# DigITs-AIML/MMNN_STS

Hardware: AMD Instinct MI355X
Metric: training volumes/sec/GPU (128^3 T1+T2+preop, batch 2) at 1/2/4/8 MI355X (higher is better)
Workload: dtype f32; 1 GPU; configs[2] --images --preop --survival --blend: MultiModalModel(DenseNet121-3D(in=2), MLP(32), blend) fwd + GradientBlender Cox loss + bwd + grad all-reduce + SGD-Nesterov/OneCycle step, dropout 0.2; micro_batch=2, global_batch=2, tabular=32, parallelism=dp1, allreduce=none

## Files before the change

### mmnn_sts_amd/csrc/densenet.hip

```cpp
#include "densenet.hpp"

#include <string.h>

#include <algorithm>

#include "fprop.hpp"
#include "stem.hpp"
#include "wgrad.hpp"

namespace mmnn {

constexpr size_t KZ_PART_BYTES = (size_t)512 * 4 * 1024 * sizeof(float);
constexpr unsigned KZ_CNT_ENTRIES = 4096;

namespace {
struct Panel { const float* p; unsigned bytes; };
struct LayerBind {
  BnFwd bn1, bn2;
  BnBwd gr_new, gr_t1;
  StatPtr dg1, dg2, s_x;
  View x, g;
  View x_new, g_new;
  View t1, dz2;
};
}

static long conv1_elems(const Plan& p, int cin) { return (long)p.mid * cin; }
static long conv2_elems(const Plan& p) { return (long)p.cfg.growth * p.mid * 27; }
static long trans_elems(const TransOff& t) { return (long)t.cout * t.cin; }
static size_t conv2_split_bytes(const Plan& p) { return (size_t)3 * conv2_elems(p) * sizeof(uint16_t); }

int plan_build(Plan& p, const NetCfg& cfg, int N, int D, int H, int W) {
  MMNN_REQUIRE(cfg.nblocks >= 1 && cfg.nblocks <= MAX_BLOCKS, "plan: 1..%d dense blocks supported, got %d", MAX_BLOCKS, cfg.nblocks);
  MMNN_REQUIRE(cfg.in_channels >= 1 && cfg.in_channels <= 4, "plan: in_channels must be 1..4, got %d", cfg.in_channels);
  MMNN_REQUIRE(cfg.init_features >= 1 && cfg.init_features <= 64, "plan: init_features must be <= 64, got %d", cfg.init_features);
  MMNN_REQUIRE(cfg.growth >= 1 && cfg.growth <= 32, "plan: growth_rate must be <= 32, got %d", cfg.growth);
  MMNN_REQUIRE(cfg.bn_size >= 1 && cfg.dropout_p >= 0.f && cfg.dropout_p < 1.f, "plan: bad bn_size / dropout");
  MMNN_REQUIRE(N >= 1 && D >= 1 && H >= 1 && W >= 1, "plan: bad input extent");
  p.cfg = cfg; p.N = N; p.D = D; p.H = H; p.W = W;
  p.mid = cfg.bn_size * cfg.growth;
  p.D0 = (D - 1) / 2 + 1; p.H0 = (H - 1) / 2 + 1; p.W0 = (W - 1) / 2 + 1;
  int d = (p.D0 - 1) / 2 + 1, h = (p.H0 - 1) / 2 + 1, w = (p.W0 - 1) / 2 + 1;
  int c = cfg.init_features;
  for (int b = 0; b < cfg.nblocks; ++b) {
    MMNN_REQUIRE(cfg.block_layers[b] >= 1, "plan: empty dense block %d", b);
    MMNN_REQUIRE(d >= 1 && h >= 1 && w >= 1, "plan: input too small, block %d has no voxels", b + 1);
    p.Db[b] = d; p.Hb[b] = h; p.Wb[b] = w; p.Vb[b] = d * h * w;
    p.cin_b[b] = c;
    p.nrep_b[b] = (b == 0 || (long)N * d * h * w >= 32768) ? NREP : ((long)N * d * h * w >= 4096 ? 2 : 1);
    p.ctot_b[b] = c + cfg.block_layers[b] * cfg.growth;
    c = p.ctot_b[b];
    if (b != cfg.nblocks - 1) {
      MMNN_REQUIRE(c % 2 == 0, "plan: transition halves an odd channel count");
      c /= 2; d /= 2; h /= 2; w /= 2;
    }
  }
  long po = 0, ro = 0;
  int nbn = 0;
  auto bn = [&](int ch, long& w_, long& b_, long& m_, long& v_) { w_ = po; po += ch; b_ = po; po += ch; m_ = ro; ro += ch; v_ = ro; ro += ch; ++nbn; };
  p.p_conv0 = po; po += (long)cfg.init_features * cfg.in_channels * 343;
  bn(cfg.init_features, p.p_n0w, p.p_n0b, p.r_n0m, p.r_n0v);
  p.layers.assign(cfg.nblocks, {});
  p.trans.clear();
  for (int b = 0; b < cfg.nblocks; ++b) {
    int ci = p.cin_b[b];
    for (int l = 0; l < cfg.block_layers[b]; ++l) {
      LayerOff lo;
      lo.cin = ci;
      bn(ci, lo.n1w, lo.n1b, lo.r1m, lo.r1v);
      lo.c1 = po; po += conv1_elems(p, ci);
      bn(p.mid, lo.n2w, lo.n2b, lo.r2m, lo.r2v);
      lo.c2 = po; po += conv2_elems(p);
      p.layers[b].push_back(lo);
      ci += cfg.growth;
    }
    if (b != cfg.nblocks - 1) {
      TransOff t;
      t.cin = ci; t.cout = ci / 2;
      bn(ci, t.nw, t.nb, t.rm, t.rv);
      t.cw = po; po += trans_elems(t);
      p.trans.push_back(t);
    } else {
      bn(ci, p.p_n5w, p.p_n5b, p.r_n5m, p.r_n5v);
    }
  }
  p.n_params = po; p.n_runstats = ro; p.n_bn = nbn;

  Carver cv;
  const int nb = cfg.nblocks;
  const size_t F = sizeof(float);
  const long V0 = (long)p.D0 * p.H0 * p.W0;
  p.o_conv0 = cv.take((size_t)N * cfg.init_features * V0 * F);
  p.o_idx = cv.take((size_t)N * cfg.init_features * p.Vb[0]);
  p.o_t1.assign(nb, {});
  size_t dap = 0;
  for (int b = 0; b < nb; ++b) {
    p.o_x[b] = cv.take((size_t)N * p.ctot_b[b] * p.Vb[b] * F);
    p.o_g[b] = cv.take((size_t)N * p.ctot_b[b] * p.Vb[b] * F);
    for (int l = 0; l < cfg.block_layers[b]; ++l) p.o_t1[b].push_back(cv.take((size_t)N * p.mid * p.Vb[b] * F));
    if (b != nb - 1) {
      p.o_ap[b] = cv.take((size_t)N * p.ctot_b[b] * p.Vb[b + 1] * F);
      dap = std::max(dap, (size_t)N * p.ctot_b[b] * p.Vb[b + 1] * F);
    } else {
      p.o_ap[b] = 0;
    }
  }
  p.o_dap = cv.take(dap ? dap : 256);
  p.o_dz0 = cv.take((size_t)N * cfg.init_features * V0 * F);
  const size_t PAIR = 2 * NREP * sizeof(double);
  p.o_fstat = cv.cur;
  p.o_st_conv0 = cv.take(PAIR * cfg.init_features);
  p.o_st_t1.assign(nb, {});
  for (int b = 0; b < nb; ++b) {
    p.o_st_x[b] = cv.take(PAIR * p.ctot_b[b]);
    for (int l = 0; l < cfg.block_layers[b]; ++l) p.o_st_t1[b].push_back(cv.take(PAIR * p.mid));
  }
  p.fstat_bytes = cv.cur - p.o_fstat;
  p.o_bstat = cv.cur;
  p.o_dg_n0 = cv.take(PAIR * cfg.init_features);
  p.o_dg_n1.assign(nb, {}); p.o_dg_n2.assign(nb, {}); p.o_dg_tr.clear();
  for (int b = 0; b < nb; ++b) {
    p.o_s_x[b] = cv.take(PAIR * p.ctot_b[b]);
    for (int l = 0; l < cfg.block_layers[b]; ++l) {
      p.o_dg_n1[b].push_back(cv.take(PAIR * p.layers[b][l].cin));
      p.o_dg_n2[b].push_back(cv.take(PAIR * p.mid));
    }
    if (b != nb - 1) p.o_dg_tr.push_back(cv.take(PAIR * p.ctot_b[b]));
  }
  p.o_dg_n5 = cv.take(PAIR * p.ctot_b[nb - 1]);
  p.bstat_bytes = cv.cur - p.o_bstat;
  p.o_pk_conv0 = cv.take((size_t)7 * stem_krows(cfg.in_channels) * 64 * F);
  p.o_pk_c1.assign(nb, {}); p.o_pk_c2f.assign(nb, {}); p.o_pk_c2b.assign(nb, {}); p.o_pk_tr.clear();
  p.o_pk_c2f3.assign(nb, {}); p.o_pk_c2b3.assign(nb, {});
  p.x3_bytes = 0;
  for (int b = 0; b < nb; ++b) {
    FpropArgs f, g;
    memset(&f, 0, sizeof(f));
    f.N = N; f.D = p.Db[b]; f.H = p.Hb[b]; f.W = p.Wb[b];
    g = f;
    f.Cin = p.mid; f.M = cfg.growth;
    g.Cin = cfg.growth; g.M = p.mid;
    const bool f3 = conv3_fwd_bf16x3_eligible(f), b3 = conv3_dgrad_bf16x3_eligible(g);
    if (f3) p.x3_bytes = std::max(p.x3_bytes, conv3_bf16x3_plane_bytes(f));
    if (b3) p.x3_bytes = std::max(p.x3_bytes, conv3_bf16x3_plane_bytes(g));
    for (int l = 0; l < cfg.block_layers[b]; ++l) {
      p.o_pk_c1[b].push_back(cv.take(conv1_elems(p, p.layers[b][l].cin) * F));
      p.o_pk_c2f[b].push_back(cv.take(conv2_elems(p) * F));
      p.o_pk_c2b[b].push_back(cv.take(conv2_elems(p) * F));
      p.o_pk_c2f3[b].push_back(f3 ? cv.take(conv2_split_bytes(p)) : 0);
      p.o_pk_c2b3[b].push_back(b3 ? cv.take(conv2_split_bytes(p)) : 0);
    }
    if (b != nb - 1) p.o_pk_tr.push_back(cv.take(trans_elems(p.trans[b]) * F));
  }
  p.o_x3 = p.x3_bytes ? cv.take(p.x3_bytes) : 0;
  p.ns_conv0 = stem_wgrad_pick_splits(N, p.D0, p.H0, p.W0, cfg.in_channels);
  p.o_sl_conv0 = cv.take((size_t)p.ns_conv0 * cfg.in_channels * cfg.init_features * 352 * F);
  p.o_sl_c1.assign(nb, {}); p.o_sl_c2.assign(nb, {}); p.ns_c1.assign(nb, {}); p.ns_c2.assign(nb, {});
  p.o_sl_tr.clear(); p.ns_tr.clear();
  for (int b = 0; b < nb; ++b) {
    for (int l = 0; l < cfg.block_layers[b]; ++l) {
      const int ci = p.layers[b][l].cin;
      int pairs = 0;
      {
        const int cw = wgrad1_channel_width(ci, p.Vb[b]);
        for (int k = 0; k < cfg.block_layers[b]; ++k)
          if (wgrad1_channel_width(p.layers[b][k].cin, p.Vb[b]) == cw) pairs += cdiv(p.layers[b][k].cin, cw);
      }
      const int s1 = wgrad_pick_splits(1, N, p.Db[b], p.Hb[b], p.Wb[b], p.mid, ci, pairs);
      const int s2 = wgrad_pick_splits(27, N, p.Db[b], p.Hb[b], p.Wb[b], cfg.growth, p.mid, cfg.block_layers[b]);
      p.ns_c1[b].push_back(s1); p.ns_c2[b].push_back(s2);
      p.o_sl_c1[b].push_back(cv.take(s1 * conv1_elems(p, ci) * F));
      p.o_sl_c2[b].push_back(cv.take(s2 * conv2_elems(p) * F));
    }
    if (b != nb - 1) {
      const int s = wgrad_pick_splits(1, N, p.Db[b + 1], p.Hb[b + 1], p.Wb[b + 1], p.trans[b].cout, p.trans[b].cin);
      p.ns_tr.push_back(s);
      p.o_sl_tr.push_back(cv.take(s * trans_elems(p.trans[b]) * F));
    }
  }
  for (int b = 0; b < nb; ++b) p.o_dz2[b] = cv.take((size_t)cfg.block_layers[b] * N * p.mid * p.Vb[b] * F);
  p.o_kz_part = cv.take(KZ_PART_BYTES);
  p.o_kz_cnt = cv.take(KZ_CNT_ENTRIES * sizeof(unsigned));
  int nlayers = 0;
  for (int b = 0; b < nb; ++b) nlayers += cfg.block_layers[b];
  p.n_run_jobs = nbn;
  p.n_pack_jobs = 1 + 5 * nlayers + (nb - 1);
  p.n_grad_jobs = 3 + 6 * nlayers + 3 * (nb - 1) + 2;
  p.o_jobs_run = cv.take(sizeof(RunStatJob) * p.n_run_jobs);
  p.o_jobs_pack = cv.take(sizeof(PackJob) * p.n_pack_jobs);
  p.o_jobs_grad = cv.take(sizeof(GradJob) * p.n_grad_jobs);
  p.n_layers = nlayers;
  p.o_wg_table = cv.take(sizeof(WgradArgs) * 2 * nlayers);
  p.ws_bytes = cv.cur;
  p.host_jobs_bytes = p.o_wg_table - p.o_jobs_run;
  if (p.host_jobs) { (void)hipHostFree(p.host_jobs); p.host_jobs = nullptr; }
  p.tab_params = nullptr; p.tab_run = nullptr; p.tab_ws = nullptr;
  return 0;
}

void plan_free(Plan& p) {
  if (p.host_jobs) (void)hipHostFree(p.host_jobs);
  p.host_jobs = nullptr;
  if (p.wg_pinned) (void)hipHostFree(p.wg_pinned);
  p.wg_pinned = nullptr;
  for (hipEvent_t e : p.timer_ev) (void)hipEventDestroy(e);
  p.timer_ev.clear();
}

static NormSite concat_site(const Plan& p, int b, int C, long w, long bb, long rm, long rv, size_t o_dg) {
  return {p.o_st_x[b], p.o_s_x[b], o_dg, p.ctot_b[b], 0, C, p.nrep_b[b], w, bb, rm, rv, (double)p.N * p.Vb[b]};
}
static NormSite norm0(const Plan& p) {
  const int C = p.cfg.init_features;
  return {p.o_st_conv0, p.o_dg_n0, p.o_dg_n0, C, 0, C, NREP, p.p_n0w, p.p_n0b, p.r_n0m, p.r_n0v, (double)p.N * p.D0 * p.H0 * p.W0};
}
static NormSite norm1(const Plan& p, int b, int l) {
  const LayerOff& lo = p.layers[b][l];
  return concat_site(p, b, lo.cin, lo.n1w, lo.n1b, lo.r1m, lo.r1v, p.o_dg_n1[b][l]);
}
static NormSite norm2(const Plan& p, int b, int l) {
  const LayerOff& lo = p.layers[b][l];
  return {p.o_st_t1[b][l], p.o_dg_n2[b][l], p.o_dg_n2[b][l], p.mid, 0, p.mid, p.nrep_b[b], lo.n2w, lo.n2b, lo.r2m, lo.r2v, (double)p.N * p.Vb[b]};
}
static NormSite transition(const Plan& p, int b) {
  const TransOff& t = p.trans[b];
  return concat_site(p, b, t.cin, t.nw, t.nb, t.rm, t.rv, p.o_dg_tr[b]);
}
static NormSite norm5(const Plan& p) {
  const int b = p.cfg.nblocks - 1;
  return concat_site(p, b, p.ctot_b[b], p.p_n5w, p.p_n5b, p.r_n5m, p.r_n5v, p.o_dg_n5);
}

static StatPtr statptr(char* ws, size_t o, int C, int off, int nrep) {
  StatPtr s; memset(&s, 0, sizeof(s));
  s.sum = reinterpret_cast<double*>(ws + o); s.sq = s.sum + (long)NREP * C;
  s.stride = C; s.off = off; s.nrep = nrep;
  return s;
}
static StatPtr stats(char* ws, const NormSite& s, int first = 0, int training = 1) {
  StatPtr st = statptr(ws, s.o_st, s.stride, s.off + first, s.nrep);
  if (!training) st.sum = nullptr;
  return st;
}
static StatPtr sums(char* ws, const NormSite& s, int first = 0) { return statptr(ws, s.o_s, s.stride, s.off + first, s.nrep); }
static StatPtr dgsums(char* ws, const NormSite& s) { return statptr(ws, s.o_dg, s.C, 0, s.nrep); }
static BnFwd bnfwd(const Plan& p, char* ws, const float* params, float* run, const NormSite& s, int training) {
  BnFwd f; memset(&f, 0, sizeof(f));
  f.st = stats(ws, s);
  f.rmean = run + s.rm; f.rvar = run + s.rv; f.gamma = params + s.w; f.beta = params + s.b;
  f.inv_count = 1.0 / s.count; f.eps = p.cfg.eps; f.training = training;
  return f;
// ... 313 lines not shown
  set_x(w2, L.t1); w2.bn = L.bn2;
  w2.slab = fptr(ws, p.o_sl_c2[b][l]); w2.slab_stride = conv2_elems(p); w2.nsplit = p.ns_c2[b][l];
  wgrad_shape(w1, p, b);
  w1.M = p.mid; w1.Cin = cin;
  set_g0(w1, L.dz2); set_g1(w1, L.t1); w1.gr = L.gr_t1;
  set_x(w1, L.x); w1.bn = L.bn1;
  w1.slab = fptr(ws, p.o_sl_c1[b][l]); w1.slab_stride = conv1_elems(p, cin); w1.nsplit = p.ns_c1[b][l];
}

static ConsumerBwdArgs consumer_bwd_args(const Plan& p, const float* params, float* run, char* ws, const NormSite& s, int b, int mode, const float* dy) {
  const View X = concat(p, ws, b), G = concat_grad(p, ws, b);
  const StatPtr dg = dgsums(ws, s);
  ConsumerBwdArgs a; memset(&a, 0, sizeof(a));
  a.N = p.N; a.C = s.C; a.D = p.Db[b]; a.H = p.Hb[b]; a.W = p.Wb[b]; a.mode = mode; a.nrep = s.nrep;
  a.dy = dy; a.x = X.p; a.x_ns = X.ns;
  a.bn = bnfwd(p, ws, params, run, s, 1);
  a.g = G.p; a.g_ns = G.ns; a.dbeta = dg.sum; a.dgamma = dg.sq;
  a.s_acc = sums(ws, s);
  return a;
}

int plan_backward(Plan& p, const float* params, const float* x, char* ws, const float* grad_out, float* grad_params, int accumulate,
                  uint64_t seed, hipStream_t stream) {
  return plan_backward_range(p, params, x, ws, grad_out, grad_params, accumulate, seed, p.cfg.nblocks - 1, 0, stream);
}

int plan_block_param_range(const Plan& p, int block, long* begin, long* end) {
  const int nb = p.cfg.nblocks;
  MMNN_REQUIRE(block >= -1 && block < nb && begin && end, "block_param_range: block %d out of range [-1, %d)", block, nb);
  if (block < 0) { *begin = 0; *end = norm1(p, 0, 0).w; return 0; }
  *begin = norm1(p, block, 0).w;
  *end = (block + 1 < nb) ? norm1(p, block + 1, 0).w : p.n_params;
  return 0;
}

int plan_backward_range(Plan& p, const float* params, const float* x, char* ws, const float* grad_out, float* grad_params, int accumulate,
                        uint64_t seed, int hi, int lo, hipStream_t stream) {
  MMNN_REQUIRE(params && x && ws && grad_out && grad_params, "backward: null buffer");
  MMNN_REQUIRE(p.tab_ws == ws && p.tab_params == params, "backward: must follow a training forward on the same buffers");
  const NetCfg& c = p.cfg;
  const int nb = c.nblocks, N = p.N;
  MMNN_REQUIRE(hi >= lo && lo >= 0 && hi < nb, "backward: bad block range [%d, %d] of %d blocks", lo, hi, nb);
  MMNN_REQUIRE(hi == nb - 1 || p.bwd_next == hi, "backward: block range [%d, %d] out of order (expected to continue at block %d)", lo, hi, p.bwd_next);
  float* run = p.tab_run;
  int rc;
  const bool first_call = hi == nb - 1;
  if (first_call) {
    MMNN_HIP(hipMemsetAsync(ws + p.o_bstat, 0, p.bstat_bytes, stream));
    MMNN_HIP(hipMemsetAsync(ws + p.o_kz_cnt, 0, KZ_CNT_ENTRIES * sizeof(unsigned), stream));
  }
  p.bwd_next = lo - 1;
  if (first_call || !p.wg_uploaded) {
    const size_t bytes = sizeof(WgradArgs) * 2 * p.n_layers;
    if (!p.wg_pinned) {
      MMNN_HIP(hipHostMalloc(&p.wg_pinned, bytes, hipHostMallocDefault));
      p.wg_shadow.assign(bytes, 0);
      p.wg_uploaded = false;
    }
    std::vector<WgradArgs> tab(2 * p.n_layers);
    int id = 0;
    for (int b = 0; b < nb; ++b)
      for (int l = 0; l < c.block_layers[b]; ++l, ++id) {
        layer_wgrad_args(p, layer_bind(p, params, run, ws, b, l), ws, b, l, id, tab[id], tab[p.n_layers + id]);
        tab[id].trace = trace_slot(p);
        tab[p.n_layers + id].trace = trace_slot(p);
      }
    if (!p.wg_uploaded || memcmp(tab.data(), p.wg_shadow.data(), bytes) != 0) {
      if (p.wg_uploaded) MMNN_HIP(hipStreamSynchronize(stream));
      memcpy(p.wg_pinned, tab.data(), bytes);
      memcpy(p.wg_shadow.data(), tab.data(), bytes);
      MMNN_HIP(hipMemcpyAsync(ws + p.o_wg_table, p.wg_pinned, bytes, hipMemcpyHostToDevice, stream));
      p.wg_uploaded = true;
    }
  }
  const WgradArgs* dev_w2 = reinterpret_cast<const WgradArgs*>(ws + p.o_wg_table);
  const WgradArgs* dev_w1 = dev_w2 + p.n_layers;
  const WgradArgs* host_w2 = static_cast<const WgradArgs*>(p.wg_pinned);
  const WgradArgs* host_w1 = host_w2 + p.n_layers;
  auto block_wgrads = [&](int b, int id0) -> int {
    const int np = c.block_layers[b];
    int rc2;
    { ScopedTimer t(p, T_CONV2_WGRAD, b, stream); rc2 = launch_wgrad_batched(host_w2 + id0, dev_w2 + id0, np, seed, 27, PRO_BNRELU, stream); }
    if (rc2) return rc2;
    for (int j = id0 + np; j > id0;) {
      int i = j - 1;
      while (i > id0 && wgrad1_channel_width(host_w1[i - 1].Cin, p.Vb[b]) == wgrad1_channel_width(host_w1[j - 1].Cin, p.Vb[b])) --i;
      {
        ScopedTimer t(p, T_CONV1_WGRAD, b, stream);
        rc2 = j - i > 1 ? launch_wgrad_batched(host_w1 + i, dev_w1 + i, j - i, seed, 1, PRO_BNRELU, stream)
                        : launch_wgrad1(host_w1[i], PRO_BNRELU, stream);
      }
      if (rc2) return rc2;
      j = i;
    }
    return 0;
  };
  if (first_call && (rc = launch_consumer_bwd(consumer_bwd_args(p, params, run, ws, norm5(p), nb - 1, 0, grad_out), stream))) return rc;
  int layer_id = 0;
  for (int b = 0; b <= hi; ++b) layer_id += c.block_layers[b];
  for (int b = hi; b >= lo; --b) {
    for (int l = c.block_layers[b] - 1; l >= 0; --l) {
      --layer_id;
      const LayerBind L = layer_bind(p, params, run, ws, b, l);
      const int cin = p.layers[b][l].cin;
      FpropArgs a = block_args(p, ws, b);
      a.Cin = c.growth; a.M = p.mid;
      set_in0(a, L.g_new); set_in1(a, L.x_new); a.gr_in = L.gr_new;
      a.drop_in = dropcfg(p, seed, layer_id, 1);
      set_conv2_weights(a, p, ws, b, l, true); a.w_ld = p.mid;
      set_out(a, L.dz2); set_ex(a, L.t1); a.ebn = L.bn2;
      a.dbeta = L.dg2.sum; a.dgamma = L.dg2.sq;
      prefetch(a, conv1_weights(p, params, b, l));
      { ScopedTimer t(p, T_CONV2_DGRAD, b, stream); rc = launch_fprop(a, 27, PRO_GRAD, EPI_MASK_STORE, stream); }
      if (rc) return rc;
      FpropArgs d = block_args(p, ws, b);
      d.Cin = p.mid; d.M = cin;
      set_in0(d, L.dz2); set_in1(d, L.t1); d.gr_in = L.gr_t1;
      d.w = conv1_weights(p, params, b, l).p; d.w_ld = cin;
      set_out(d, L.g); set_ex(d, L.x); d.ebn = L.bn1;
      d.dbeta = L.dg1.sum; d.dgamma = L.dg1.sq;
      d.s_acc = L.s_x;
      if (l > 0) prefetch(d, conv2_panel(p, ws, b, l - 1, true));
      { ScopedTimer t(p, T_CONV1_DGRAD, b, stream); rc = launch_fprop(d, 1, PRO_GRAD, EPI_MASK_ACCUM, stream); }
      if (rc) return rc;
    }
    if ((rc = block_wgrads(b, layer_id))) return rc;
    const View X = concat(p, ws, b), G = concat_grad(p, ws, b);
    const BnBwd gr = bnbwd(p, ws, params, norm1(p, b, 0));
    if (b > 0) {
      const int pb = b - 1;
      const TransOff& t = p.trans[pb];
      WgradArgs w;
      wgrad_shape(w, p, b);
      w.M = t.cout; w.Cin = t.cin;
      set_g0(w, G); set_g1(w, X); w.gr = gr;
      set_x(w, pooled(p, ws, pb));
      w.slab = fptr(ws, p.o_sl_tr[pb]); w.slab_stride = trans_elems(t); w.nsplit = p.ns_tr[pb];
      if ((rc = launch_wgrad1(w, PRO_NONE, stream))) return rc;
      FpropArgs d = block_args(p, ws, b);
      d.nrep = 0;
      d.Cin = t.cout; d.M = t.cin;
      set_in0(d, G); set_in1(d, X); d.gr_in = gr;
      d.w = params + t.cw; d.w_ld = t.cin;
      set_out(d, pooled_grad(p, ws, pb));
      if ((rc = launch_fprop(d, 1, PRO_GRAD, EPI_STORE, stream))) return rc;
      if ((rc = launch_consumer_bwd(consumer_bwd_args(p, params, run, ws, transition(p, pb), pb, 1, pooled_grad(p, ws, pb).p), stream))) return rc;
    } else {
      const NormSite n0 = norm0(p);
      const StatPtr dg = dgsums(ws, n0);
      StemPoolBwdArgs q; memset(&q, 0, sizeof(q));
      q.N = N; q.C = c.init_features; q.Di = p.D0; q.Hi = p.H0; q.Wi = p.W0; q.Do = p.Db[0]; q.Ho = p.Hb[0]; q.Wo = p.Wb[0];
      q.x = fptr(ws, p.o_conv0);
      q.bn = bnfwd(p, ws, params, run, n0, 1);
      q.g = G.p; q.g_ns = G.ns; q.xp = X.p; q.xp_ns = X.ns;
      q.gr = gr;
      q.idx = reinterpret_cast<const unsigned char*>(ws + p.o_idx);
      q.dz = fptr(ws, p.o_dz0);
      q.dbeta = dg.sum; q.dgamma = dg.sq;
      if ((rc = launch_stem_pool_bwd(q, stream))) return rc;
      StemWgradArgs w; memset(&w, 0, sizeof(w));
      w.N = N; w.Cin = c.in_channels; w.D = p.D; w.H = p.H; w.W = p.W; w.Do = p.D0; w.Ho = p.H0; w.Wo = p.W0; w.M = c.init_features;
      w.x = x; w.dz = fptr(ws, p.o_dz0); w.y = fptr(ws, p.o_conv0);
      w.gr = bnbwd(p, ws, params, n0);
      w.slab = fptr(ws, p.o_sl_conv0); w.slab_stride = (long)c.in_channels * c.init_features * 352; w.nsplit = p.ns_conv0;
      { ScopedTimer t(p, T_STEM_WGRAD, -1, stream); rc = launch_stem_wgrad(w, stream); }
      if (rc) return rc;
    }
  }
  const long stem_count = (long)c.init_features * c.in_channels * 343;
  const GradJob* jobs = reinterpret_cast<const GradJob*>(ws + p.o_jobs_grad);
  const int j0 = lo == 0 ? 0 : p.gj_begin[lo], j1 = p.gj_begin[hi + 1];
  long jmax = lo == 0 ? stem_count : 0;
  for (int b = lo; b <= hi; ++b) jmax = std::max(jmax, p.gj_max[b]);
// ... 52 lines not shown
```

### mmnn_sts_amd/csrc/wgrad.hip

```cpp
#include "wgrad.hpp"

#include <algorithm>

namespace mmnn {

static void wg3_tile(int W, int& TD, int& TH, int& TW) {
  if (W > 16) { TD = 1; TH = 2; TW = 32; }
  else if (W > 8) { TD = 1; TH = 4; TW = 16; }
  else if (W > 4) { TD = 2; TH = 4; TW = 8; }
  else { TD = 4; TH = 4; TW = 4; }
}

static int wg1_wc(int Cin, long V) {
  const int thr = V >= 32768 ? 256 : 97;
  return Cin >= thr ? 8 : 4;
}

int wgrad_pick_splits(int taps, int N, int D, int H, int W, int M, int Cin, int batch) {
  if (batch < 1) batch = 1;
  if (taps == 27) {
    int TD, TH, TW;
    wg3_tile(W, TD, TH, TW);
    const long ntiles = (long)N * cdiv(D, TD) * cdiv(H, TH) * cdiv(W, TW);
    const int cgroups = cdiv(Cin, 32);
    long s = 512 / ((long)cgroups * batch);
    if (s > 64) s = 64;
    if (s > ntiles / 2) s = ntiles / 2;
    return s < 1 ? 1 : (int)s;
  }
  const long V = (long)D * H * W;
  const long nchunks = (long)N * cdiv(V, 64);
  const int wc = wg1_wc(Cin, V);
  constexpr long target = 2048;
  const long groups = (long)cdiv(Cin, 32 * wc) * cdiv(M, 128);
  long s = batch > 1 ? target / batch : target / groups;
  const long slab_cap = ((long)64 << 20) / ((long)M * Cin * 4);
  if (s > slab_cap) s = slab_cap;
  if (s > nchunks / 2) s = nchunks / 2;
  return s < 1 ? 1 : (int)s;
}

int wgrad1_channel_width(int Cin, long V) { return 32 * wg1_wc(Cin, V); }

int wgrad3_launch_batched(const WgradArgs* host, const WgradArgs* dev, int count, uint64_t seed, hipStream_t stream);
int wgrad1_launch(const WgradArgs& a, int pro_x, int wc, hipStream_t s);
int wgrad1_launch_batched(const WgradArgs* host, const WgradArgs* dev, int count, uint64_t seed, int wc, hipStream_t stream);

int launch_wgrad_batched(const WgradArgs* host, const WgradArgs* dev, int count, uint64_t seed, int taps, int pro_x, hipStream_t stream) {
  MMNN_REQUIRE(host && dev && count >= 1 && count <= 65535, "wgrad batch: bad table (count %d)", count);
  MMNN_REQUIRE(pro_x == PRO_BNRELU, "wgrad batch: only the dense-layer kernels (BN+ReLU input prologue) are batched");
  MMNN_REQUIRE(taps == 1 || taps == 27, "wgrad: taps must be 1 or 27");
  const WgradArgs& f = host[0];
  for (int i = 0; i < count; ++i) {
    const WgradArgs& a = host[i];
    MMNN_REQUIRE(a.N == f.N && a.D == f.D && a.H == f.H && a.W == f.W && a.M == f.M, "wgrad batch: layer %d differs in extent", i);
    MMNN_REQUIRE(a.N > 0 && a.D > 0 && a.H > 0 && a.W > 0 && a.Cin > 0 && a.M > 0, "wgrad: non-positive extent");
    MMNN_REQUIRE((long)a.D * a.H * a.W < (1l << 30), "wgrad: volume too large for 32-bit voxel indices");
    MMNN_REQUIRE(taps != 27 || (long)33 * a.D * a.H * a.W < (1l << 31), "wgrad: volume too large for 32-bit element offsets of a 32-channel group");
    MMNN_REQUIRE(a.g0 && a.g1 && a.x && a.slab, "wgrad: null operand");
    MMNN_REQUIRE(a.nsplit >= 1 && a.nsplit <= 65535, "wgrad: bad split count %d", a.nsplit);
    MMNN_REQUIRE(a.slab_stride >= (long)taps * a.M * a.Cin, "wgrad: slab stride too small");
    MMNN_REQUIRE(taps == 27 ? a.M <= 32 : a.M <= 128, "wgrad batch: %d output channels exceed one block row", a.M);
    MMNN_REQUIRE(taps == 27 || wg1_wc(a.Cin, (long)a.D * a.H * a.W) == wg1_wc(f.Cin, (long)f.D * f.H * f.W), "wgrad batch: layer %d needs another channel-group width", i);
  }
  if (taps == 27) return wgrad3_launch_batched(host, dev, count, seed, stream);
  return wgrad1_launch_batched(host, dev, count, seed, wg1_wc(f.Cin, (long)f.D * f.H * f.W), stream);
}

int launch_wgrad1(const WgradArgs& a, int pro_x, hipStream_t stream) {
  MMNN_REQUIRE(a.N > 0 && a.D > 0 && a.H > 0 && a.W > 0 && a.Cin > 0 && a.M > 0, "wgrad: non-positive extent");
  MMNN_REQUIRE((long)a.D * a.H * a.W < (1l << 30), "wgrad: volume too large for 32-bit voxel indices");
  MMNN_REQUIRE(a.g0 && a.g1 && a.x && a.slab, "wgrad: null operand");
  MMNN_REQUIRE(a.nsplit >= 1 && a.nsplit <= 65535, "wgrad: bad split count %d", a.nsplit);
  MMNN_REQUIRE(a.slab_stride >= (long)a.M * a.Cin, "wgrad: slab stride too small");
  MMNN_REQUIRE(pro_x == PRO_BNRELU || pro_x == PRO_NONE, "wgrad: unsupported input prologue %d", pro_x);
  return wgrad1_launch(a, pro_x, wg1_wc(a.Cin, (long)a.D * a.H * a.W), stream);
}

}
```

### mmnn_sts_amd/csrc/wgrad.hpp

```cpp
#pragma once
#include <type_traits>

#include "common.hpp"
#include "fprop.hpp"

namespace mmnn {

struct WgradArgs {
  int N, D, H, W;
  int M, Cin;
  const float* g0; long g0_ns; int g0_coff;
  const float* g1; long g1_ns; int g1_coff;
  BnBwd gr;
  DropCfg drop;
  const float* x; long x_ns; int x_coff;
  BnFwd bn;
  float* slab; long slab_stride; int nsplit;
  unsigned long long* trace;
};

int launch_wgrad1(const WgradArgs& a, int pro_x, hipStream_t stream);
int launch_wgrad_batched(const WgradArgs* host, const WgradArgs* dev_table, int count, uint64_t seed, int taps, int pro_x, hipStream_t stream);
int wgrad1_channel_width(int Cin, long V);
int wgrad_pick_splits(int taps, int N, int D, int H, int W, int M, int Cin, int batch = 1);

#if defined(__HIPCC__)

#if !defined(MMNN_TRACE_TID)
#define MMNN_TRACE_TID 0
#endif

#define MMNN_GLOBAL __attribute__((address_space(1)))

template <int TD, int TH, int TW>
struct Wg3Cfg {
  static constexpr int VT = TD * TH * TW;
  static constexpr int RS = TW + 2, HS = TH + 2, DS = TD + 2;
  static constexpr int XS = (DS * HS * RS) | 1;
  static constexpr int YS = VT + 1;
  static constexpr int NTHREADS = 8 * 64;
  static_assert(VT == 64, "tile must hold 64 voxels (two per MFMA k-step, 32 steps)");
  static_assert(32 % TW == 0, "tile width must divide 32");
  static constexpr int STAGE = 32 * XS + 32 * YS;
  static size_t smem_bytes() { return sizeof(float) * (2 * STAGE + 3 * 32 + 2 * 32 + 3 * 32); }
};

template <int NTP, int TD, int TH, int TW, class F>
__device__ __forceinline__ void wg3_mfma(f32x16 (&acc)[4], const float* yl, const float* x0, const float* x1, const float* x2, const float* x3, F&& filler) {
  constexpr int RS = Wg3Cfg<TD, TH, TW>::RS, HS = Wg3Cfg<TD, TH, TW>::HS;
  float a0, a1, b0[4], b1[4];
  auto rd = [&](int s, float& av, float (&bv)[4]) {
    const int wx = s % TW, hy = (s / TW) % TH, dz = s / (TW * TH);
    const int p0 = (dz * HS + hy) * RS + wx;
    av = yl[s];
    bv[0] = x0[p0]; bv[1] = x1[p0]; bv[2] = x2[p0];
    if (NTP == 4) bv[3] = x3[p0];
  };
  auto mm = [&](float av, const float (&bv)[4]) {
    acc[0] = __builtin_amdgcn_mfma_f32_32x32x2f32(av, bv[0], acc[0], 0, 0, 0);
    acc[1] = __builtin_amdgcn_mfma_f32_32x32x2f32(av, bv[1], acc[1], 0, 0, 0);
    acc[2] = __builtin_amdgcn_mfma_f32_32x32x2f32(av, bv[2], acc[2], 0, 0, 0);
    if (NTP == 4) acc[3] = __builtin_amdgcn_mfma_f32_32x32x2f32(av, bv[3], acc[3], 0, 0, 0);
  };
  rd(0, a0, b0);
#pragma unroll
  for (int s = 0; s < 32; s += 2) {
    rd(s + 1, a1, b1);
    __builtin_amdgcn_sched_group_barrier(0x100, NTP + 1, 0);
    mm(a0, b0);
    __builtin_amdgcn_sched_group_barrier(0x008, NTP, 0);
    filler(s);
    if (s + 2 < 32) rd(s + 2, a0, b0);
    __builtin_amdgcn_sched_group_barrier(0x100, NTP + 1, 0);
    mm(a1, b1);
    __builtin_amdgcn_sched_group_barrier(0x008, NTP, 0);
    filler(s + 1);
  }
}

template <int PRO_X, int TD, int TH, int TW>
__device__ __forceinline__ void wgrad3_body(const WgradArgs& a, const int split, const int cg) {
  using C = Wg3Cfg<TD, TH, TW>;
  constexpr int RS = C::RS, HS = C::HS, DS = C::DS, XS = C::XS, YS = C::YS, NTHREADS = C::NTHREADS;
  extern __shared__ __attribute__((aligned(16))) float smem[];
  float* Xs = smem;
  float* Ys = Xs + 32 * XS;
  float* gcoef = smem + 2 * C::STAGE;
  float* xcoef = gcoef + 96;
  float* gbase = xcoef + 64;
  const int tid = threadIdx.x, lane = tid & 63, wave = tid >> 6, half = lane >> 5, l31 = lane & 31;
  const int V = a.D * a.H * a.W;
  const int c0 = cg * 32;
  const int nw = (a.W + TW - 1) / TW, nh = (a.H + TH - 1) / TH, nd = (a.D + TD - 1) / TD;
  const int tiles_per_n = nw * nh * nd;
  const int ntiles = a.N * tiles_per_n;
  const int t_begin = (int)((long)ntiles * split / a.nsplit), t_end = (int)((long)ntiles * (split + 1) / a.nsplit);

  auto coefficients = [&]() {
    if (tid < 32) {
      float ca = 0.f, cb = 0.f, mu, rs;
      if (PRO_X == PRO_BNRELU && c0 + tid < a.Cin) bn_fwd_coef(a.bn, c0 + tid, ca, cb, mu, rs);
      xcoef[tid] = ca; xcoef[32 + tid] = cb;
      float p = 0.f, q = 0.f, r = 0.f;
      if (tid < a.M) bn_bwd_coef(a.gr, tid, p, q, r);
      gbase[tid] = p; gbase[32 + tid] = q; gbase[64 + tid] = r;
    }
  };
// ... 558 lines not shown
```

Baseline: 260.1 volumes/s (whole job; 1 volume = 1 patient = stacked T1+T2 2x128^3 + 32 tabular).

## Add bf16x3 MFMA kernel for 1x1 conv weight-gradient in large-volume blocks

Adds a new batched weight-gradient kernel for the 1x1 bottleneck convolutions. It splits the f32 gradient and activation operands into three bf16 parts and accumulates six bf16 MFMA products, keeping near-fp32 accuracy while using matrix cores. The kernel applies the BN-backward/dropout and BN+ReLU prologues while staging into double-buffered LDS. It is enabled by default for M=128, Cin a multiple of 32 up to 256, and W>16, which covers only the first dense block at this input size. Split counts and layer grouping are adjusted so eligible layers batch into one launch. The trade-offs are extra MFMA work from the split products and a large LDS footprint per workgroup.

```diff
diff --git a/mmnn_sts_amd/csrc/conv1_bf16x3.hip b/mmnn_sts_amd/csrc/conv1_bf16x3.hip
--- /dev/null
+++ b/mmnn_sts_amd/csrc/conv1_bf16x3.hip
@@ -0,0 +1,229 @@
+#include <stdlib.h>
+
+#include <algorithm>
+
+#include "bf16x3.hpp"
+#include "wgrad.hpp"
+
+namespace mmnn {
+
+typedef float f32x16_t __attribute__((ext_vector_type(16)));
+typedef __bf16 bf16x8_t __attribute__((ext_vector_type(8)));
+
+namespace c1b {
+constexpr int WG_MAXC = 256;
+constexpr int WG_VK = 32;
+constexpr int WG_WAVES = 8;
+
+__device__ __forceinline__ bf16x8_t as_bf16x8(uint4 v) { return __builtin_bit_cast(bf16x8_t, v); }
+
+__device__ __forceinline__ void mma6_split(f32x16_t& big, f32x16_t& small, const bf16x8_t (&a)[3], const bf16x8_t (&b)[3]) {
+  small = __builtin_amdgcn_mfma_f32_32x32x16_bf16(a[1], b[1], small, 0, 0, 0);
+  small = __builtin_amdgcn_mfma_f32_32x32x16_bf16(a[0], b[2], small, 0, 0, 0);
+  small = __builtin_amdgcn_mfma_f32_32x32x16_bf16(a[2], b[0], small, 0, 0, 0);
+  small = __builtin_amdgcn_mfma_f32_32x32x16_bf16(a[0], b[1], small, 0, 0, 0);
+  small = __builtin_amdgcn_mfma_f32_32x32x16_bf16(a[1], b[0], small, 0, 0, 0);
+  big = __builtin_amdgcn_mfma_f32_32x32x16_bf16(a[0], b[0], big, 0, 0, 0);
+}
+
+static int bf16x3_mode() {
+  static const int mode = [] { const char* e = getenv("MMNN_BF16X3"); return e ? atoi(e) : 32; }();
+  return mode;
+}
+}
+
+namespace c1b {
+__host__ __device__ constexpr int wg_rows(int Cin) { return 128 + Cin + 4; }
+static size_t wg_smem(int Cin) { return (size_t)2 * 3 * 4 * wg_rows(Cin) * 16; }
+
+template <int NCT>
+__device__ __forceinline__ void wgrad1_bf16x3_body(const WgradArgs& a, const int split, uint4* lds) {
+  constexpr int RPT = WG_WAVES * 16, NA = 128 / RPT, NB = (32 * NCT + RPT - 1) / RPT;
+  constexpr int HS = WG_WAVES / 4, NJ = (NCT + HS - 1) / HS;
+  const int tid = threadIdx.x, lane = tid & 63, wv = tid >> 6, mt = wv & 3, hs = wv >> 2;
+  const int V = a.D * a.H * a.W, Cin = a.Cin, R = wg_rows(Cin);
+  const int chunks_per_n = (V + WG_VK - 1) / WG_VK, nchunks = a.N * chunks_per_n;
+  const int k_begin = (int)((long)nchunks * split / a.nsplit), k_end = (int)((long)nchunks * (split + 1) / a.nsplit);
+  const int k8 = tid & 3, r0 = tid >> 2;
+  const MMNN_GLOBAL float* g0p = (const MMNN_GLOBAL float*)a.g0;
+  const MMNN_GLOBAL float* g1p = (const MMNN_GLOBAL float*)a.g1;
+  const MMNN_GLOBAL float* xp = (const MMNN_GLOBAL float*)a.x;
+  f32x4 ga[NA][2], gb[NA][2], xb[NB][2];
+  unsigned ok_lo = 0, ok_hi = 0;
+  int ld_n = -1;
+  auto load_chunk = [&](int ch) {
+    const int n = ch / chunks_per_n, v = (ch % chunks_per_n) * WG_VK + 8 * k8;
+    ok_lo = v < V; ok_hi = v + 4 < V;
+    const int o0 = ok_lo ? v : 0, o1 = ok_hi ? v + 4 : 0;
+    ld_n = n;
+#pragma unroll
+    for (int i = 0; i < NA; ++i) {
+      const long row0 = (long)n * a.g0_ns + (long)(a.g0_coff + r0 + RPT * i) * V, row1 = (long)n * a.g1_ns + (long)(a.g1_coff + r0 + RPT * i) * V;
+      ga[i][0] = *reinterpret_cast<const MMNN_GLOBAL f32x4*>(g0p + row0 + o0);
+      ga[i][1] = *reinterpret_cast<const MMNN_GLOBAL f32x4*>(g0p + row0 + o1);
+      gb[i][0] = *reinterpret_cast<const MMNN_GLOBAL f32x4*>(g1p + row1 + o0);
+      gb[i][1] = *reinterpret_cast<const MMNN_GLOBAL f32x4*>(g1p + row1 + o1);
+    }
+#pragma unroll
+    for (int i = 0; i < NB; ++i) {
+      const int c = r0 + RPT * i;
+      const long row = (long)n * a.x_ns + (long)(a.x_coff + (c < Cin ? c : 0)) * V;
+      xb[i][0] = *reinterpret_cast<const MMNN_GLOBAL f32x4*>(xp + row + o0);
+      xb[i][1] = *reinterpret_cast<const MMNN_GLOBAL f32x4*>(xp + row + o1);
+    }
+  };
+  if (k_begin < k_end) load_chunk(k_begin);
+  float bp[NA], bq[NA], br[NA], cp[NA], cq[NA], cr[NA], xa[NB], xc[NB];
+#pragma unroll
+  for (int i = 0; i < NA; ++i) bn_bwd_coef(a.gr, r0 + RPT * i, bp[i], bq[i], br[i]);
+#pragma unroll
+  for (int i = 0; i < NB; ++i) {
+    float mu, rs;
+    xa[i] = 0.f; xc[i] = 0.f;
+    if (r0 + RPT * i < Cin) bn_fwd_coef(a.bn, r0 + RPT * i, xa[i], xc[i], mu, rs);
+  }
+  int st_n = -1;
+  auto store_chunk = [&](uint4* buf) {
+    if (ld_n != st_n) {
+#pragma unroll
+      for (int i = 0; i < NA; ++i) {
+        const float sc = drop_scale(a.drop, ld_n, r0 + RPT * i);
+        cp[i] = bp[i] * sc; cq[i] = bq[i] * sc; cr[i] = br[i] * sc;
+      }
+      st_n = ld_n;
+    }
+    uint4* dst = buf + k8 * R;
+#pragma unroll
+    for (int i = 0; i < NA; ++i) {
+      float t[8];
+#pragma unroll
+      for (int e = 0; e < 8; ++e) {
+        const float v = fmaf(cp[i], ga[i][e >> 2][e & 3], fmaf(cq[i], gb[i][e >> 2][e & 3], cr[i]));
+        t[e] = ((e < 4) ? ok_lo : ok_hi) ? v : 0.f;
+      }
+      uint4 hi, mid, lo;
+      split3x8(t, hi, mid, lo);
+      const int row = r0 + RPT * i;
+      dst[row] = hi; dst[4 * R + row] = mid; dst[8 * R + row] = lo;
+    }
+#pragma unroll
+    for (int i = 0; i < NB; ++i) {
+      const int c = r0 + RPT * i;
+      if (c < Cin) {
+        float t[8];
+#pragma unroll
+        for (int e = 0; e < 8; ++e) {
+          const float v = fmaxf(fmaf(xa[i], xb[i][e >> 2][e & 3], xc[i]), 0.f);
+          t[e] = ((e < 4) ? ok_lo : ok_hi) ? v : 0.f;
+        }
+        uint4 hi, mid, lo;
+        split3x8(t, hi, mid, lo);
+        dst[128 + c] = hi; dst[4 * R + 128 + c] = mid; dst[8 * R + 128 + c] = lo;
+      }
+    }
+  };
+  f32x16_t acc[NJ], acs[NJ];
+#pragma unroll
+  for (int j = 0; j < NJ; ++j)
+#pragma unroll
+    for (int q = 0; q < 16; ++q) { acc[j][q] = 0.f; acs[j][q] = 0.f; }
+  if (k_begin < k_end) {
+    store_chunk(lds);
+    if (k_begin + 1 < k_end) load_chunk(k_begin + 1);
+  }
+  __syncthreads();
+  for (int ch = k_begin; ch < k_end; ++ch) {
+    const uint4* cur = lds + ((ch - k_begin) & 1) * (12 * R);
+    if (ch + 1 < k_end) {
+      store_chunk(lds + (((ch - k_begin) & 1) ^ 1) * (12 * R));
+      if (ch + 2 < k_end) load_chunk(ch + 2);
+    }
+#pragma unroll
+    for (int ks = 0; ks < 2; ++ks) {
+      const uint4* src = cur + (2 * ks + (lane >> 5)) * R + (lane & 31);
+      bf16x8_t af[3];
+#pragma unroll
+      for (int p = 0; p < 3; ++p) af[p] = as_bf16x8(src[p * 4 * R + mt * 32]);
+#pragma unroll
+      for (int jj = 0; jj < NJ; ++jj) {
+        const int j = jj * HS + hs;
+        if (j < NCT) {
+          bf16x8_t bf[3];
+#pragma unroll
+          for (int p = 0; p < 3; ++p) bf[p] = as_bf16x8(src[p * 4 * R + 128 + 32 * j]);
+          mma6_split(acc[jj], acs[jj], af, bf);
+        }
+      }
+    }
+    __syncthreads();
+  }
+  float* out = a.slab + (long)split * a.slab_stride;
+#pragma unroll
+  for (int jj = 0; jj < NJ; ++jj) {
+    const int j = jj * HS + hs;
+    if (j < NCT) {
+#pragma unroll
+      for (int q = 0; q < 16; ++q) {
+        const int m = mt * 32 + 8 * (q / 4) + 4 * (lane >> 5) + q % 4;
+        out[(long)m * Cin + 32 * j + (lane & 31)] = acc[jj][q] + acs[jj][q];
+      }
+    }
+  }
+}
+}
+
+__global__ void __launch_bounds__(c1b::WG_WAVES * 64) wgrad1_bf16x3_batched_kernel(const WgradArgs* __restrict__ table, const int count, const uint64_t seed) {
+  extern __shared__ uint4 c1b_lds[];
+  WgradArgs a = table[count - 1 - (int)blockIdx.y];
+  const int split = blockIdx.x;
+  if (split >= a.nsplit) return;
+  a.drop.seed = seed;
+  switch (a.Cin / 32) {
+    case 1: c1b::wgrad1_bf16x3_body<1>(a, split, c1b_lds); break;
+    case 2: c1b::wgrad1_bf16x3_body<2>(a, split, c1b_lds); break;
+    case 3: c1b::wgrad1_bf16x3_body<3>(a, split, c1b_lds); break;
+    case 4: c1b::wgrad1_bf16x3_body<4>(a, split, c1b_lds); break;
+    case 5: c1b::wgrad1_bf16x3_body<5>(a, split, c1b_lds); break;
+    case 6: c1b::wgrad1_bf16x3_body<6>(a, split, c1b_lds); break;
+    case 7: c1b::wgrad1_bf16x3_body<7>(a, split, c1b_lds); break;
+    case 8: c1b::wgrad1_bf16x3_body<8>(a, split, c1b_lds); break;
+    default: break;
+  }
+}
+
+bool wgrad1_bf16x3_shape(int N, int D, int H, int W, int M, int Cin) {
+  const long V = (long)D * H * W;
+  return c1b::bf16x3_mode() != 0 && N > 0 && M == 128 && Cin >= 32 && Cin % 32 == 0 && Cin <= c1b::WG_MAXC && W > 16 && V % 4 == 0;
+}
+bool wgrad1_bf16x3_eligible(const WgradArgs& a) {
+  return wgrad1_bf16x3_shape(a.N, a.D, a.H, a.W, a.M, a.Cin) && a.g0 && a.g1 && a.x && a.slab &&
+         (((uintptr_t)a.g0 | (uintptr_t)a.g1 | (uintptr_t)a.x) & 15) == 0 && ((a.g0_ns | a.g1_ns | a.x_ns) & 3) == 0;
+}
+int wgrad1_bf16x3_splits(int N, long V, int batch) {
+  const long nchunks = (long)N * cdiv(V, c1b::WG_VK);
+  long s = 512 / (batch < 1 ? 1 : batch);
+  if (s > nchunks / 2) s = nchunks / 2;
+  return s < 1 ? 1 : (int)s;
+}
+
+int wgrad1_bf16x3_launch_batched(const WgradArgs* host, const WgradArgs* dev, int count, uint64_t seed, hipStream_t stream) {
+  int gx = 1, cmax = 0;
+  for (int i = 0; i < count; ++i) {
+    MMNN_REQUIRE(wgrad1_bf16x3_eligible(host[i]), "wgrad1 bf16x3: layer %d not handled (M=%d, Cin=%d, W=%d)", i, host[i].M, host[i].Cin, host[i].W);
+    gx = std::max(gx, host[i].nsplit);
+    cmax = std::max(cmax, host[i].Cin);
+  }
+  const size_t smem = c1b::wg_smem(cmax);
+  MMNN_REQUIRE(smem <= 160 * 1024, "wgrad1 bf16x3: %zu bytes of LDS", smem);
+  static size_t configured[MAX_DEVICES] = {0};
+  size_t& conf = configured[current_device_slot()];
+  if (smem > conf) {
+    MMNN_HIP(hipFuncSetAttribute(reinterpret_cast<const void*>(wgrad1_bf16x3_batched_kernel), hipFuncAttributeMaxDynamicSharedMemorySize, (int)smem));
+    conf = smem;
+  }
+  MMNN_LAUNCH(wgrad1_bf16x3_batched_kernel, dim3((unsigned)gx, (unsigned)count), dim3(c1b::WG_WAVES * 64), smem, stream, dev, count, seed);
+  MMNN_HIP(hipGetLastError());
+  return 0;
+}
+
+}
diff --git a/mmnn_sts_amd/csrc/densenet.hip b/mmnn_sts_amd/csrc/densenet.hip
--- a/mmnn_sts_amd/csrc/densenet.hip
+++ b/mmnn_sts_amd/csrc/densenet.hip
@@ -29,6 +29,7 @@
 static long conv2_elems(const Plan& p) { return (long)p.cfg.growth * p.mid * 27; }
 static long trans_elems(const TransOff& t) { return (long)t.cout * t.cin; }
 static size_t conv2_split_bytes(const Plan& p) { return (size_t)3 * conv2_elems(p) * sizeof(uint16_t); }
+static bool conv1_wgrad3(const Plan& p, int b, int cin) { return wgrad1_bf16x3_shape(p.N, p.Db[b], p.Hb[b], p.Wb[b], p.mid, cin); }
 
 int plan_build(Plan& p, const NetCfg& cfg, int N, int D, int H, int W) {
   MMNN_REQUIRE(cfg.nblocks >= 1 && cfg.nblocks <= MAX_BLOCKS, "plan: 1..%d dense blocks supported, got %d", MAX_BLOCKS, cfg.nblocks);
@@ -161,12 +162,16 @@
     for (int l = 0; l < cfg.block_layers[b]; ++l) {
       const int ci = p.layers[b][l].cin;
       int pairs = 0;
+      const bool w3 = conv1_wgrad3(p, b, ci);
       {
         const int cw = wgrad1_channel_width(ci, p.Vb[b]);
-        for (int k = 0; k < cfg.block_layers[b]; ++k)
-          if (wgrad1_channel_width(p.layers[b][k].cin, p.Vb[b]) == cw) pairs += cdiv(p.layers[b][k].cin, cw);
+        for (int k = 0; k < cfg.block_layers[b]; ++k) {
+          const int ck = p.layers[b][k].cin;
+          if (conv1_wgrad3(p, b, ck)) pairs += w3 ? 1 : 0;
+          else if (!w3 && wgrad1_channel_width(ck, p.Vb[b]) == cw) pairs += cdiv(ck, cw);
+        }
       }
-      const int s1 = wgrad_pick_splits(1, N, p.Db[b], p.Hb[b], p.Wb[b], p.mid, ci, pairs);
+      const int s1 = wgrad_pick_splits(1, N, p.Db[b], p.Hb[b], p.Wb[b], p.mid, ci, pairs, w3);
       const int s2 = wgrad_pick_splits(27, N, p.Db[b], p.Hb[b], p.Wb[b], cfg.growth, p.mid, cfg.block_layers[b]);
       p.ns_c1[b].push_back(s1); p.ns_c2[b].push_back(s2);
       p.o_sl_c1[b].push_back(cv.take(s1 * conv1_elems(p, ci) * F));
@@ -646,13 +651,14 @@
     int rc2;
     { ScopedTimer t(p, T_CONV2_WGRAD, b, stream); rc2 = launch_wgrad_batched(host_w2 + id0, dev_w2 + id0, np, seed, 27, PRO_BNRELU, stream); }
     if (rc2) return rc2;
+    auto cls = [&](int k) { return wgrad1_bf16x3_eligible(host_w1[k]) ? 0 : wgrad1_channel_width(host_w1[k].Cin, p.Vb[b]); };
     for (int j = id0 + np; j > id0;) {
       int i = j - 1;
-      while (i > id0 && wgrad1_channel_width(host_w1[i - 1].Cin, p.Vb[b]) == wgrad1_channel_width(host_w1[j - 1].Cin, p.Vb[b])) --i;
+      while (i > id0 && cls(i - 1) == cls(j - 1)) --i;
       {
         ScopedTimer t(p, T_CONV1_WGRAD, b, stream);
-        rc2 = j - i > 1 ? launch_wgrad_batched(host_w1 + i, dev_w1 + i, j - i, seed, 1, PRO_BNRELU, stream)
-                        : launch_wgrad1(host_w1[i], PRO_BNRELU, stream);
+        rc2 = (j - i > 1 || cls(i) == 0) ? launch_wgrad_batched(host_w1 + i, dev_w1 + i, j - i, seed, 1, PRO_BNRELU, stream)
+                                         : launch_wgrad1(host_w1[i], PRO_BNRELU, stream);
       }
       if (rc2) return rc2;
       j = i;
diff --git a/mmnn_sts_amd/csrc/wgrad.hip b/mmnn_sts_amd/csrc/wgrad.hip
--- a/mmnn_sts_amd/csrc/wgrad.hip
+++ b/mmnn_sts_amd/csrc/wgrad.hip
@@ -16,7 +16,10 @@
   return Cin >= thr ? 8 : 4;
 }
 
-int wgrad_pick_splits(int taps, int N, int D, int H, int W, int M, int Cin, int batch) {
+int wgrad1_bf16x3_splits(int N, long V, int batch);
+int wgrad1_bf16x3_launch_batched(const WgradArgs* host, const WgradArgs* dev, int count, uint64_t seed, hipStream_t stream);
+
+int wgrad_pick_splits(int taps, int N, int D, int H, int W, int M, int Cin, int batch, bool bf16x3) {
   if (batch < 1) batch = 1;
   if (taps == 27) {
     int TD, TH, TW;
@@ -29,6 +32,7 @@
     return s < 1 ? 1 : (int)s;
   }
   const long V = (long)D * H * W;
+  if (bf16x3 && wgrad1_bf16x3_shape(N, D, H, W, M, Cin)) return wgrad1_bf16x3_splits(N, V, batch);
   const long nchunks = (long)N * cdiv(V, 64);
   const int wc = wg1_wc(Cin, V);
   constexpr long target = 2048;
@@ -51,6 +55,8 @@
   MMNN_REQUIRE(pro_x == PRO_BNRELU, "wgrad batch: only the dense-layer kernels (BN+ReLU input prologue) are batched");
   MMNN_REQUIRE(taps == 1 || taps == 27, "wgrad: taps must be 1 or 27");
   const WgradArgs& f = host[0];
+  bool all3 = taps == 1;
+  for (int i = 0; i < count && all3; ++i) all3 = wgrad1_bf16x3_eligible(host[i]);
   for (int i = 0; i < count; ++i) {
     const WgradArgs& a = host[i];
     MMNN_REQUIRE(a.N == f.N && a.D == f.D && a.H == f.H && a.W == f.W && a.M == f.M, "wgrad batch: layer %d differs in extent", i);
@@ -61,9 +67,10 @@
     MMNN_REQUIRE(a.nsplit >= 1 && a.nsplit <= 65535, "wgrad: bad split count %d", a.nsplit);
     MMNN_REQUIRE(a.slab_stride >= (long)taps * a.M * a.Cin, "wgrad: slab stride too small");
     MMNN_REQUIRE(taps == 27 ? a.M <= 32 : a.M <= 128, "wgrad batch: %d output channels exceed one block row", a.M);
-    MMNN_REQUIRE(taps == 27 || wg1_wc(a.Cin, (long)a.D * a.H * a.W) == wg1_wc(f.Cin, (long)f.D * f.H * f.W), "wgrad batch: layer %d needs another channel-group width", i);
+    MMNN_REQUIRE(taps == 27 || all3 || wg1_wc(a.Cin, (long)a.D * a.H * a.W) == wg1_wc(f.Cin, (long)f.D * f.H * f.W), "wgrad batch: layer %d needs another channel-group width", i);
   }
   if (taps == 27) return wgrad3_launch_batched(host, dev, count, seed, stream);
+  if (all3) return wgrad1_bf16x3_launch_batched(host, dev, count, seed, stream);
   return wgrad1_launch_batched(host, dev, count, seed, wg1_wc(f.Cin, (long)f.D * f.H * f.W), stream);
 }
 
diff --git a/mmnn_sts_amd/csrc/wgrad.hpp b/mmnn_sts_amd/csrc/wgrad.hpp
--- a/mmnn_sts_amd/csrc/wgrad.hpp
+++ b/mmnn_sts_amd/csrc/wgrad.hpp
@@ -22,7 +22,9 @@
 int launch_wgrad1(const WgradArgs& a, int pro_x, hipStream_t stream);
 int launch_wgrad_batched(const WgradArgs* host, const WgradArgs* dev_table, int count, uint64_t seed, int taps, int pro_x, hipStream_t stream);
 int wgrad1_channel_width(int Cin, long V);
-int wgrad_pick_splits(int taps, int N, int D, int H, int W, int M, int Cin, int batch = 1);
+int wgrad_pick_splits(int taps, int N, int D, int H, int W, int M, int Cin, int batch = 1, bool bf16x3 = false);
+bool wgrad1_bf16x3_shape(int N, int D, int H, int W, int M, int Cin);
+bool wgrad1_bf16x3_eligible(const WgradArgs& a);
 
 #if defined(__HIPCC__)
 
```

After: 262.0 volumes/s (whole job; 1 volume = 1 patient = stacked T1+T2 2x128^3 + 32 tabular) (median of 6 runs). No clear change (+0.7%).
